# Francesco215/autoregressive_diffusion

Measured on AMD Instinct MI355X. Metric: denoiser-step frames/sec at 1/2/4/8 MI355X; 64-frame Lunar-Lander seq, higher is better.
Workload: dtype bf16; 1 GPU; Lunar-Lander 64-frame seq, gym EDM2 UNet 46.2M (gym_train.py:37-47), 8 seq/GPU (gym_train.py:55 micro_batch_size), step = EDM2Loss fwd + bwd + grad all-reduce + [grad-norm clip +] AdamW + 2 EMA profiles, 3:1 mix of 3-D/2-D steps; global_batch=8, seq_len=64, parallelism=dp1, hip_graph=False

## Files before the change

### autoregressive_diffusion_amd/_lib.py

```python
import ctypes as C
import os

import torch

_HERE = os.path.dirname(os.path.abspath(__file__))
LIB_PATH = os.path.join(_HERE, os.environ.get("ONIRIS_LIB_NAME", "liboniris_hip.so"))

if not os.path.exists(LIB_PATH):
    raise ImportError(f"{LIB_PATH} not found: build the HIP extension first (make -j8 at the repo root); "
                      "there is no CPU/PyTorch fallback for the denoiser kernels")

lib = C.CDLL(LIB_PATH)

c_void_p, c_int, c_float, c_int32, c_int64, c_size_t = C.c_void_p, C.c_int, C.c_float, C.c_int32, C.c_int64, C.c_size_t


class WeightDesc(C.Structure):
    _fields_ = [("w", c_void_p), ("grad", c_void_p), ("wf", c_void_p), ("wb", c_void_p), ("dwp", c_void_p), ("dws", c_void_p),
                ("cout", c_int32), ("cin", c_int32), ("taps", c_int32), ("kt", c_int32),
                ("CoutP", c_int32), ("CinP", c_int32), ("CoutPb", c_int32), ("CinPb", c_int32),
                ("row_start", c_int32), ("perm3", c_int32), ("gain", c_float), ("nsplit_cap", c_int32),
                ("nsplit", c_void_p), ("tile_start", c_int32), ("pad_", c_int32)]


class ConvArgs(C.Structure):
    _fields_ = [("x", c_void_p), ("ctx", c_void_p), ("w_own", c_void_p), ("w_ctx", c_void_p), ("out", c_void_p),
                ("coef_own", c_void_p), ("coef_ctx", c_void_p),
                ("B", c_int32), ("S", c_int32), ("T", c_int32), ("H", c_int32), ("W", c_int32),
                ("Cin", c_int32), ("CinP", c_int32), ("Cout", c_int32), ("CoutP", c_int32), ("taps", c_int32),
                ("ctx_bstride", c_int32), ("ctx_T", c_int32), ("coff0", c_int32), ("coff1", c_int32),
                ("ctx_fill", c_float), ("epi", c_int32),
                ("res", c_void_p), ("escale", c_void_p), ("emb_gain", c_void_p), ("out2", c_void_p),
                ("ta", c_float), ("tb", c_float), ("clip", c_float), ("ctx_out", c_void_p),
                ("big_tile", c_int32), ("escale_pitch", c_int32),
                ("splitk_ws", c_void_p), ("splitk_ws_bytes", C.c_size_t), ("clip_flag", c_void_p),
                ("ctx_prod", c_void_p), ("ctx_prod_mode", c_int32), ("x_split", c_int32), ("x2", c_void_p), ("act_out", c_void_p),
                ("cat_w1", c_float), ("cat_w2", c_float), ("ctx_rows", c_int32)]


class WgradArgs(C.Structure):
    _fields_ = [("x", c_void_p), ("dy", c_void_p), ("dwp", c_void_p), ("scale", c_void_p),
                ("B", c_int32), ("T", c_int32), ("H", c_int32), ("W", c_int32), ("Cin", c_int32), ("CinP", c_int32),
                ("Cout", c_int32), ("CoutP", c_int32), ("taps", c_int32),
                ("xb_stride", c_int32), ("x_T", c_int32), ("coff", c_int32), ("fill", c_float),
                ("nsplit_cap", c_int32), ("taps_total", c_int32), ("tap0", c_int32), ("pad_", c_int32),
                ("nsplit_out", c_void_p)]


class AttnArgs(C.Structure):
    _fields_ = [("q", c_void_p), ("k", c_void_p), ("v", c_void_p), ("qt", c_void_p), ("kt", c_void_p),
                ("vt", c_void_p), ("out", c_void_p), ("lse", c_void_p),
                ("kv_num", c_void_p), ("kv_idx", c_void_p), ("q_num", c_void_p), ("q_idx", c_void_p),
                ("tab_cols", c_int32), ("qtab_cols", c_int32),
                ("B", c_int32), ("heads", c_int32), ("Lq", c_int32), ("Lk", c_int32), ("C", c_int32),
                ("mask_mode", c_int32), ("P", c_int32), ("T", c_int32), ("tab_block", c_int32),
                ("dout", c_void_p), ("doutt", c_void_p), ("delta", c_void_p),
                ("dq", c_void_p), ("dk", c_void_p), ("dv", c_void_p),
                ("dkv_part", c_void_p), ("dkv_chunks", c_int32), ("dkv_item_keys", c_int32),
                ("sched", c_void_p), ("sched_wgs", c_int32), ("sched_slots", c_int32), ("v_bstride", c_int64),
                ("k_bstride", c_int64), ("split_ws", c_void_p), ("kv_splits", c_int32), ("frame_kernel", c_int32)]


class AttnF32Args(C.Structure):
    _fields_ = [("q", c_void_p), ("k", c_void_p), ("v", c_void_p), ("out", c_void_p), ("lse", c_void_p),
                ("dout", c_void_p), ("delta", c_void_p), ("dq", c_void_p), ("dk", c_void_p), ("dv", c_void_p),
                ("BH", c_int32), ("Lq", c_int32), ("Lk", c_int32), ("D", c_int32), ("mask_mode", c_int32), ("P", c_int32),
                ("T", c_int32), ("q_frame_off", c_int32), ("scale", c_float), ("pad_", c_int32)]


EPI_NONE, EPI_EMB_SILU, EPI_MPSUM = 0, 1, 2

_SIGS = {
    "oniris_last_error": (C.c_char_p, []),
    "oniris_abi_version": (c_int, []),
    "oniris_struct_sizes": (c_int, [c_void_p]),
    "oniris_profile_arm": (c_int, [c_void_p, c_void_p]),
    "oniris_profile_disarm": (c_int, []),
    "oniris_set_cu_reserve": (c_int, [c_int]),
    "oniris_set_ew_nt_bytes": (c_int64, [c_int64]),
    "oniris_frame_attn_bwd": (c_int, [c_void_p, c_void_p]),
    "oniris_frame_attn_qkv_fwd": (c_int, [c_void_p, c_void_p, c_void_p, c_int64, c_int, c_int, c_void_p]),
    "oniris_frame_attn_qkv_bwd": (c_int, [c_void_p, c_void_p, c_void_p, c_void_p, c_void_p, c_int64, c_int, c_int, c_void_p]),
    "oniris_conv_f32": (c_int, [c_void_p, c_void_p, c_void_p, c_int64, c_int, c_int, c_int, c_int, c_int, c_void_p]),
    "oniris_wgrad_f32": (c_int, [c_void_p, c_void_p, c_void_p, c_int64, c_int, c_int, c_int, c_int, c_int, c_void_p]),
    "oniris_attn_f32_fwd": (c_int, [c_void_p, c_void_p]),
    "oniris_attn_f32_bwd": (c_int, [c_void_p, c_void_p]),
    "oniris_census": (c_int, [c_int]),
    "oniris_census_read": (c_int64, [C.c_char_p, c_int64]),
    "oniris_train_mask": (c_int, [c_int, c_int, c_void_p, c_void_p, C.POINTER(c_int)]),
    "oniris_infer_mask": (c_int, [c_int, c_int, c_void_p, c_void_p, C.POINTER(c_int)]),
    "oniris_mask_transpose": (c_int, [c_int, c_int, c_void_p, c_void_p, c_void_p, c_void_p]),
    "oniris_attn_schedule": (c_int, [c_int, c_int, c_void_p, c_int, c_void_p, c_int]),
    "oniris_weight_prep": (c_int, [c_void_p, c_int, c_int, c_int, c_int, c_void_p]),
# ... 131 lines not shown
```

### autoregressive_diffusion_amd/csrc/common.h

```cpp
#pragma once
#include <hip/hip_runtime.h>
#include <hip/hip_ext.h>
#include <stdint.h>
#include <stdio.h>
#include <string.h>

typedef __bf16 bf16;
typedef __attribute__((ext_vector_type(8))) __bf16 bf16x8;
typedef __attribute__((ext_vector_type(4))) __bf16 bf16x4;
typedef __attribute__((ext_vector_type(2))) __bf16 bf16x2;
typedef __attribute__((ext_vector_type(4))) short s16x4;
typedef __attribute__((ext_vector_type(16))) float f32x16;
typedef __attribute__((ext_vector_type(4))) float f32x4;
typedef __attribute__((ext_vector_type(4))) unsigned int u32x4;

#define ONIRIS_OK 0
#define ONIRIS_EINVAL (-1)
#define ONIRIS_ELAUNCH (-2)
#define ONIRIS_EUNSUPPORTED (-3)

void oniris_set_error(const char* fmt, ...);

#define ONIRIS_CHECK_ARG(cond, ...)                \
  do {                                             \
// ... 46 lines not shown
}
template <bool NT, typename V>
__device__ __forceinline__ void stv(V* p, V v) {
  if constexpr (NT) __builtin_nontemporal_store(v, p);
  else *p = v;
}

extern int oniris_cu_reserve;
int oniris_persistent_wgs(void);

static inline int cdiv(int a, int b) { return (a + b - 1) / b; }
static inline int roundup(int a, int b) { return cdiv(a, b) * b; }

#ifdef __HIPCC__
__device__ __forceinline__ float bf2f(bf16 v) { return (float)v; }
__device__ __forceinline__ bf16 f2bf(float v) { return (bf16)v; }

__device__ __forceinline__ f32x16 mfma32(bf16x8 a, bf16x8 b, f32x16 c) {
  return __builtin_amdgcn_mfma_f32_32x32x16_bf16(a, b, c, 0, 0, 0);
}
__device__ __forceinline__ float sigmoid_fast(float z) {
  return __builtin_amdgcn_rcpf(1.f + __builtin_amdgcn_exp2f(-1.4426950408889634f * z));
}
__device__ __forceinline__ int mfma_row(int r, int lane) { return (r & 3) + 8 * (r >> 2) + 4 * (lane >> 5); }

__device__ __forceinline__ float wave_sum(float v) {
#pragma unroll
  for (int o = 32; o > 0; o >>= 1) v += __shfl_xor(v, o);
  return v;
}
__device__ __forceinline__ float wave_max(float v) {
#pragma unroll
  for (int o = 32; o > 0; o >>= 1) v = fmaxf(v, __shfl_xor(v, o));
  return v;
}

__device__ __forceinline__ float block_sum(float v, float* red) {
  v = wave_sum(v);
  const int w = threadIdx.x >> 6, nw = blockDim.x >> 6;
  __syncthreads();
  if ((threadIdx.x & 63) == 0) red[w] = v;
  __syncthreads();
  float t = 0.f;
  for (int i = 0; i < nw; ++i) t += red[i];
  return t;
}
// ... 2 lines not shown
```

### autoregressive_diffusion_amd/csrc/conv1x1_glds.h

```cpp
#pragma once
#include "conv_kernels.h"
#include "lds_dma.h"

struct C1Cfg {
  static constexpr int BM = 256, BN = 128, CK = 64, NW = 8, NTHR = 512, NSTG = 3;
  static constexpr int STG = (BM + BN) * 128;
  static constexpr int NPA = BM * 8 / NTHR, NPW = BN * 8 / NTHR;
  static constexpr int EROW = 64 * 2 + 16;
  static_assert(NW * 32 * EROW <= STG, "the epilogue stages through one (free) stage buffer");
  static_assert(NSTG * STG <= 160 * 1024, "stages must fit the LDS");
};

__global__ __launch_bounds__(512, 1) void conv1x1_glds_kernel(const ConvDev d) {
#if defined(__HIP_DEVICE_COMPILE__)
  using Cfg = C1Cfg;
  constexpr int BM = Cfg::BM, BN = Cfg::BN, CK = Cfg::CK, NTHR = Cfg::NTHR, STG = Cfg::STG, NSTG = Cfg::NSTG;
  constexpr int NPA = Cfg::NPA, NPW = Cfg::NPW, EROW = Cfg::EROW;
  __shared__ __attribute__((aligned(16))) unsigned char smem[NSTG * STG];
  const OnirisConvArgs& a = d.a;
  const int tid = threadIdx.x, lane = tid & 63, wave = __builtin_amdgcn_readfirstlane(tid >> 6), r = lane & 31, h = lane >> 5;
  const int wp = wave & 3, wc = wave >> 2;
  const int Cin = a.Cin, Cout = a.Cout;
  const long long M = (long long)a.B * a.S * a.T * a.H * a.W;
  const int nchunk = Cin / CK, ncb = d.ncob, ntiles = d.ntt * ncb;
// ... 101 lines not shown
      const long long prow = m0 + wp * 64 + m * 32;
      auto put = [&](int nt, const float (&v)[16]) __attribute__((always_inline)) {
#pragma unroll
        for (int g = 0; g < 4; ++g) {
          bf16x4 o;
#pragma unroll
          for (int k = 0; k < 4; ++k) o[k] = f2bf(v[4 * g + k]);
          *(bf16x4*)(ep + r * EROW + (nt * 32 + 8 * g + 4 * h) * 2) = o;
        }
      };
      auto flush = [&](bf16* dst) __attribute__((always_inline)) {
#pragma unroll
        for (int it = 0; it < 4; ++it) {
          const int id = it * 64 + lane, row = id >> 3, part = id & 7;
          const int co = cow + part * 8;
          if (prow + row < M && co < Cout) {
            const u32x4 v_ = *(const u32x4*)(ep + row * EROW + part * 16);
            u32x4* o_ = (u32x4*)(dst + (size_t)(prow + row) * Cout + co);
            if (d.nt) __builtin_nontemporal_store(v_, o_); else *o_ = v_;
          }
        }
      };
      float v[16];
      if (a.epi == ONIRIS_EPI_MPSUM) {
        if (a.out2) {
#pragma unroll
          for (int nt = 0; nt < 2; ++nt) {
#pragma unroll
            for (int i = 0; i < 16; ++i) v[i] = acc[m][nt][i];
            put(nt, v);
          }
          flush((bf16*)a.out2);
        }
        const bool valid = prow + r < M;
        const size_t obase = (size_t)(prow + r) * Cout;
#pragma unroll
        for (int nt = 0; nt < 2; ++nt) {
#pragma unroll
          for (int g = 0; g < 4; ++g) {
            const int co = cow + nt * 32 + 8 * g + 4 * h;
            bf16x4 rv;
#pragma unroll
            for (int k = 0; k < 4; ++k) rv[k] = f2bf(0.f);
            if (valid && co < Cout) rv = *(const bf16x4*)((const bf16*)a.res + obase + co);
#pragma unroll
            for (int k = 0; k < 4; ++k) {
              float o = a.ta * bf2f(rv[k]) + a.tb * acc[m][nt][4 * g + k];
// ... 2 lines not shown
            }
          }
          put(nt, v);
        }
        flush(og);
      } else {
#pragma unroll
        for (int nt = 0; nt < 2; ++nt) {
#pragma unroll
          for (int i = 0; i < 16; ++i) v[i] = acc[m][nt][i];
          put(nt, v);
        }
        flush(og);
      }
    }
    drained = true;
  }
#endif
}

static inline bool conv1x1_glds_ok(const OnirisConvArgs& a) {
  const long long M = (long long)a.B * a.S * a.T * a.H * a.W;
  return a.taps == 1 && !a.ctx && a.Cin % 64 == 0 && a.CinP == a.Cin && a.Cin <= 1024 && a.Cout % 8 == 0 &&
         (a.epi == ONIRIS_EPI_NONE || a.epi == ONIRIS_EPI_MPSUM) && M >= 8192 && M * a.Cin * 2 < (1LL << 31) &&
         (long long)a.CoutP * a.CinP * 2 < (1LL << 31);
}

static int launch_conv1x1_glds(const OnirisConvArgs& a, hipStream_t stream) {
  ConvDev d;
  d.a = a;
  const long long M = (long long)a.B * a.S * a.T * a.H * a.W;
  d.ntt = (int)((M + C1Cfg::BM - 1) / C1Cfg::BM);
  d.ncob = cdiv(a.CoutP, C1Cfg::BN);
  d.ntx = d.nty = 1; d.ksplit = 1; d.reduce = 0;
  d.nt = M * a.Cout * 2 >= oniris_ew_nt_bytes();
  const long long ntiles = (long long)d.ntt * d.ncob;
  const int ncu = oniris_persistent_wgs();
  const long long nblk = ntiles < ncu ? ntiles : ncu;
  oniris_launch_tagged(d.nt ? "nt-stores" : nullptr, conv1x1_glds_kernel, dim3((unsigned)nblk), dim3(C1Cfg::NTHR), stream, d);
  ONIRIS_LAUNCH_CHECK();
  return ONIRIS_OK;
}
```

### autoregressive_diffusion_amd/csrc/conv_api.hip

```cpp
#include "conv_fwd_common.h"

extern "C" int oniris_conv_fwd(const OnirisConvArgs* args, oniris_stream_t stream_) {
  hipStream_t st = (hipStream_t)stream_;
  ONIRIS_CHECK_ARG(args && args->w_own && ((args->x && args->out) || args->ctx_prod_mode == 3), "conv_fwd: null pointer");
  const OnirisConvArgs& a = *args;
  if (a.ctx_prod_mode != 0 && !(a.S == 1 && a.ctx && a.taps == 9 && a.ctx_prod)) {
    oniris_set_error("conv_fwd: ctx_prod_mode %d is for the one-frame cached evaluation (S == 1, context path, ctx_prod given)", a.ctx_prod_mode);
    return ONIRIS_EUNSUPPORTED;
  }
  if (a.ctx_rows != 0 && !(a.S == 1 && a.T == 1 && a.ctx && a.taps == 9 && a.ctx_rows > 0 && a.B == 2 * a.ctx_rows &&
                           a.ctx_out == nullptr && a.ctx_prod_mode != 3)) {
    oniris_set_error("conv_fwd: ctx_rows %d is for the one-frame cached evaluation of a guided pair (S = T = 1, context path, "
                     "B = 2 * ctx_rows (got B = %d), no ctx_out, ctx_prod_mode != 3)", a.ctx_rows, a.B);
    return ONIRIS_EUNSUPPORTED;
  }
  ONIRIS_CHECK_ARG(a.taps == 9 || a.taps == 1, "conv_fwd: taps must be 1 or 9 (got %d)", a.taps);
  ONIRIS_CHECK_ARG(a.B > 0 && a.T > 0 && a.H > 0 && a.W > 0 && (a.S == 1 || a.S == 2), "conv_fwd: bad sizes");
  ONIRIS_CHECK_ARG(a.Cin % 8 == 0 && a.Cout % 8 == 0, "conv_fwd: Cin, Cout must be multiples of 8 (%d,%d)", a.Cin, a.Cout);
  ONIRIS_CHECK_ARG(a.CoutP % 32 == 0 && a.CinP % 64 == 0 && a.CoutP >= a.Cout && a.CinP >= a.Cin,
                   "conv_fwd: bad padded sizes CoutP=%d CinP=%d", a.CoutP, a.CinP);
  ONIRIS_CHECK_ARG(a.epi != ONIRIS_EPI_MPSUM || a.res, "conv_fwd: EPI_MPSUM needs res");
  ONIRIS_CHECK_ARG(a.epi != ONIRIS_EPI_EMB_SILU || (a.escale && a.out2), "conv_fwd: EPI_EMB_SILU needs escale/out2");
  ONIRIS_CHECK_ARG(a.x2 == nullptr || (a.taps == 1 && a.ctx == nullptr), "conv_fwd: x2 (concatenated input) is a 1x1, context-free option");
  const bool has_ctx = a.ctx != nullptr;
  ONIRIS_CHECK_ARG(!has_ctx || (a.w_ctx && a.taps == 9), "conv_fwd: context path needs w_ctx and taps == 9");
  if (a.clip_flag && (a.taps == 1 || (a.S == 1 && has_ctx))) {
    const hipError_t e = hipMemsetD32Async((hipDeviceptr_t)a.clip_flag, 1, 1, st);
    if (e != hipSuccess) { oniris_set_error("conv: clip_flag fill failed: %s", hipGetErrorString(e)); return ONIRIS_ELAUNCH; }
  }
  if (a.taps == 1) {
    ONIRIS_CHECK_ARG(a.S == 1, "conv_fwd: 1x1 variant expects S == 1 (fold slots into T)");
    return conv_dispatch_1x1(a, st);
  }
  if (a.S == 2) {
    ONIRIS_CHECK_ARG(has_ctx, "conv_fwd: S == 2 is the DART training layout and needs the context path");
    return conv_dispatch_s2ctx(a, st);
  }
  return has_ctx ? conv_dispatch_s1ctx(a, st) : conv_dispatch_s1(a, st);
}
```

### autoregressive_diffusion_amd/csrc/conv_kernels.h

```cpp
#pragma once
#include <type_traits>
#include <cstdlib>
#include "common.h"
#include "../../include/oniris.h"

template <int PW_, int NPOS_ = 128>
struct Patch {
  static constexpr int PW = PW_;
  static constexpr int NPOS = NPOS_;
  static constexpr int PH = (PW_ == 16) ? (NPOS_ / 16) : PW_;
  static constexpr int FT = NPOS_ / (PW * PH);
  static constexpr int HW = PW + 2, HH = PH + 2;
  static constexpr int HALO = FT * HH * HW;
};

struct ConvDev {
  OnirisConvArgs a;
  int ntx, nty, ntt, ncob;
  int grid3d;
  int ksplit;
  int reduce;
  int nt;
};

template <int S, int TAPS, int CK, int NT, bool HAS_CTX, int PW, int NW = 4>
struct ConvCfg {
  using P = Patch<PW, 32 * NW>;
// ... 319 lines not shown
  unsigned char* ep = smem + wave * 32 * EROW;
  auto flush = [&](bf16* dst, size_t blk) __attribute__((always_inline)) {
    constexpr int PO = BN / 8;
#pragma unroll
    for (int it = 0; it < 32 * PO / 64; ++it) {
      const int id = it * 64 + lane;
      const int row = id / PO, part = id % PO;
      const int pr = wave * 32 + row;
      bool ok;
      size_t px_;
      if constexpr (TAPS == 9) {
        const int f_ = pr / (P::PH * P::PW), yy = (pr / P::PW) % P::PH, xx = pr % P::PW;
        ok = (t0 + f_) < T;
        px_ = (size_t)(t0 + f_) * HWp + (y0 + yy) * W + (x0 + xx);
      } else {
        ok = (q0 + pr) < T * HWp;
        px_ = (size_t)(q0 + pr);
      }
      const int co = co0 + part * 8;
      if (ok && co < a.Cout) *(uint4*)(dst + (blk + px_) * a.Cout + co) = *(const uint4*)(ep + row * EROW + part * 16);
    }
  };
  bf16* og = (bf16*)a.out;
#pragma unroll
  for (int s = 0; s < S; ++s) {
    const int n = (b * S + s) * T + tloc;
    const float cown = (a.coef_own && valid) ? a.coef_own[n] : 1.f;
    float cctx = 0.f;
    if constexpr (HAS_CTX) cctx = (a.coef_ctx && valid) ? a.coef_ctx[n] : 1.f;
    const size_t blk = (size_t)(b * S + s) * T * HWp;
    const size_t obase = (blk + pix) * a.Cout;
    float v[NT][16];
#pragma unroll
    for (int nt = 0; nt < NT; ++nt)
#pragma unroll
      for (int i = 0; i < 16; ++i) {
        v[nt][i] = cown * acc[s][nt][i];
        if constexpr (HAS_CTX) v[nt][i] = __builtin_fmaf(cctx, accc[nt][i], v[nt][i]);
      }
    auto stage = [&]() __attribute__((always_inline)) {
#pragma unroll
      for (int nt = 0; nt < NT; ++nt)
#pragma unroll
        for (int g = 0; g < 4; ++g) {
          bf16x4 o;
#pragma unroll
          for (int k = 0; k < 4; ++k) o[k] = f2bf(v[nt][4 * g + k]);
          *(bf16x4*)(ep + pr * EROW + (nt * 32 + 8 * g + 4 * h) * 2) = o;
        }
    };
    if (a.epi == ONIRIS_EPI_MPSUM) {
      if (a.out2) { stage(); flush((bf16*)a.out2, blk); }
#pragma unroll
      for (int nt = 0; nt < NT; ++nt)
#pragma unroll
        for (int g = 0; g < 4; ++g) {
          const int co = co0 + nt * 32 + 8 * g + 4 * h;
          bf16x4 rv;
#pragma unroll
          for (int k = 0; k < 4; ++k) rv[k] = f2bf(0.f);
          if (valid && co < a.Cout) rv = *(const bf16x4*)((const bf16*)a.res + obase + co);
#pragma unroll
          for (int k = 0; k < 4; ++k) {
            float o = a.ta * bf2f(rv[k]) + a.tb * v[nt][4 * g + k];
            if (a.clip > 0.f) o = fminf(fmaxf(o, -a.clip), a.clip);
            v[nt][4 * g + k] = o;
          }
        }
    }
    stage();
    flush(og, blk);
    if (a.epi == ONIRIS_EPI_EMB_SILU) {
#pragma unroll
// ... 73 lines not shown
```

### autoregressive_diffusion_amd/csrc/elementwise.hip

```cpp
#include <cstdlib>
#include "common.h"
#include "../../include/oniris.h"

#define SILU_SCALE (1.0f / 0.596f)

__device__ __forceinline__ float silu_f(float z) { return z * sigmoid_fast(z); }
__device__ __forceinline__ float dsilu_f(float z) {
  const float sg = sigmoid_fast(z);
  return sg * (1.f + z * (1.f - sg));
}

template <bool NORM, bool NT>
__global__ __launch_bounds__(256) void act_fwd_kernel(const bf16* __restrict__ x, const bf16* __restrict__ skip,
                                                      bf16* __restrict__ xo, bf16* __restrict__ a,
                                                      float* __restrict__ sden, long long npix, int C1, int C2, float w1,
                                                      float w2, int rs, int Ho, int Wo) {
  const int C = C1 + C2, G = C >> 3;
  const long long gid = (long long)blockIdx.x * 256 + threadIdx.x;
  const long long pix = gid / G;
  const int cg = (int)(gid % G);
  const bool ok = pix < npix;
  float v[8];
#pragma unroll
  for (int i = 0; i < 8; ++i) v[i] = 0.f;
  if (ok) {
    const int c = cg * 8;
    bf16x8 in;
    float w;
    if (c < C1) {
      w = w1;
      if (rs == 0) in = ldv<NT>((const bf16x8*)(x + pix * C1 + c));
      else {
        const int xo_ = (int)(pix % Wo), yo_ = (int)((pix / Wo) % Ho);
// ... 945 lines not shown
```

### autoregressive_diffusion_amd/edm2/networks_edm2.py

```python
import inspect
import math
from contextlib import nullcontext
import torch
from torch import nn
import torch.nn.functional as F

from .. import ops
from .. import fp32 as _fp32
from .loss_weight import MultiNoiseLoss
from .utils import BetterModule, MPFourier, to_cl, from_cl, BF16, strip_runtime_state
from .conv import MPConv, MPCausal3DGatedConv, Gating, weights_ready, batched_gates
from .attention import FrameAttention, VideoAttention


def unwrap_ddp(m):
    return m.module if isinstance(m, torch.nn.parallel.DistributedDataParallel) else m


class Block(nn.Module):
    def __init__(self, in_channels, out_channels, emb_channels, flavor="enc", resample_mode="keep",
                 resample_filter=[1, 1], attention=False, channels_per_head=64, dropout=0, res_balance=0.3,
                 attn_balance=0.3, clip_act=256):
        super().__init__()
        self._taps = ops.resample_taps(resample_filter)
# ... 11 lines not shown
        else:
            self.attn = FrameAttention(out_channels, self.num_heads, attn_balance)

    __getstate__ = strip_runtime_state

    def _cl(self, x, emb, batch_size, c_noise, cache=None, update_cache=False, just_2d=False, skip=None, cat_w=None,
            c=None, in_slot=None, skip_slot=None, private_out=False, pair=False):
        if cache is None:
            cache = {}
        rs = self.resample_mode
        if rs != "keep" and (self._taps is not None or skip is not None or (self.flavor == "enc" and self.conv_skip is not None)):
            x, in_slot, rs = ops.resample(x, rs, in_slot, self._taps), None, "keep"
        skip_conv_done = False
        want_xs = (private_out and ops.ALIAS2 and self.training and torch.is_grad_enabled()
                   and not (self.flavor == "dec" and self.conv_skip is not None))
        if self.flavor == "enc" and self.conv_skip is not None:
            x, in_slot = self.conv_skip._cl(x, in_slot=in_slot), None
        xs = ops.GradSlot() if (want_xs and (x.requires_grad or (skip is not None and skip.requires_grad))) else None
        if self.flavor == "enc":
            x, a = ops.act(x, norm=True, in_slot=in_slot, resample=rs, xo_slot=xs)
        elif (skip is not None and self.conv_skip is not None and not self.training
              and ops.conv_cat_act_ok(x, skip, self.conv_skip.weight.pw)):
            x, a = ops.conv_cat_act(x, skip, cat_w[0], cat_w[1], self.conv_skip.weight.pw)
            skip_conv_done = True
        elif skip is not None:
            x, a = ops.act(x, skip, cat_w[0], cat_w[1], want_xo=True, in_slot=in_slot, skip_slot=skip_slot, xo_slot=xs)
        else:
            x, a = ops.act(x, want_xo=True, in_slot=in_slot, resample=rs, xo_slot=xs)
        N = x.shape[0]
        if c is None:
            c = (self.emb_linear._cl(emb).reshape(N, -1).float() * self.emb_gain + 1)
        pk = dict(pair=True) if pair else {}
        y, cache["conv_res0"] = self.conv_res0._cl(a, batch_size, c_noise, cache.get("conv_res0"), update_cache,
                                                   just_2d, cscale=c, **pk)
        if self.training and self.dropout != 0:
            y = F.dropout(y, p=self.dropout)
        if self.flavor == "dec" and self.conv_skip is not None and not skip_conv_done:
            x = self.conv_skip._cl(x)
        t = self.res_balance
        den = 1.0 / math.sqrt((1 - t) ** 2 + t ** 2)
        clip = float(self.clip_act) if self.clip_act is not None else 0.0
        x, cache["conv_res1"] = self.conv_res1._cl(y, batch_size, c_noise, cache.get("conv_res1"), update_cache, just_2d,
                                                   res=x, ta=(1 - t) * den, tb=t * den,
                                                   clip=clip if self.num_heads == 0 else 0.0,
                                                   grad_private=private_out, **pk,
                                                   **(dict(res_slot=xs, res_alias=True) if xs is not None else {}))
# ... 411 lines not shown
```

### autoregressive_diffusion_amd/ops.py

```python
import ctypes
import math
import numpy as np
import torch

from . import _lib
from ._lib import lib, check

BF16 = torch.bfloat16


_raw_stream = getattr(torch._C, "_cuda_getCurrentRawStream", None)


def _stream():
    if _raw_stream is not None:
        return ctypes.c_void_p(_raw_stream(torch.cuda.current_device()))
    return ctypes.c_void_p(torch.cuda.current_stream().cuda_stream)


def _p(t):
    return None if t is None else t.data_ptr()


def _need_gpu(*ts):
# ... 480 lines not shown
    return 16 if W >= 16 else W


def _s2ctx_family(T, H, W, Cin, CinP, CoutP, ctx_T, coff, ctx_fill):
    ok = ctx_fill in (0.0, 1.0)
    if (BIG_TILE >= 4 and ok and Cin == 32 and CinP == 64 and CoutP == 32 and W % 16 == 0 and H % 4 == 0 and ctx_T == T
            and tuple(coff) in ((-2, -1), (2, 1))):
        return "stream"
    if BIG_TILE >= 3 and ok and Cin % 32 == 0 and H % 16 == 0 and W % 16 == 0:
        return "glds16"
    if BIG_TILE >= 3 and ok and Cin % 32 == 0 and H == 8 and W == 8 and CoutP % 64 == 0:
        return "glds8"
    return "staged"


PROFILE_SHAPES = int(_os.environ.get("ONIRIS_PROFILE_SHAPES", "0"))
ALIAS2 = int(_os.environ.get("ONIRIS_ALIAS2", "1"))
CLIP_FLAG = int(_os.environ.get("ONIRIS_CLIP_FLAG", "1"))


def _conv_launch(x, ctx, w_own, w_ctx, out, coef_own, coef_ctx, B, S, T, H, W, Cin, CinP, Cout, CoutP, taps,
                 ctx_bstride=0, ctx_T=0, coff=(0, 0), ctx_fill=0.0, epi=0, res=None, escale=None, emb_gain=None,
                 out2=None, ta=0.0, tb=0.0, clip=0.0, ctx_out=None, clip_flag=None, ctx_prod=None, ctx_prod_mode=0,
                 x2=None, act_out=None, x_split=0, cat_w=(1.0, 1.0), ctx_rows=0):
    if KernelProfile.enabled:
        flops = 2.0 * B * S * T * H * W * Cout * Cin * taps
        if ctx is not None:
            flops += 2.0 * B * T * H * W * Cout * Cin * 2 * taps
        nt = 2 if CoutP % 64 == 0 else 1
        if (BIG_TILE >= 4 and S == 2 and ctx is not None and taps == 9 and Cin == 32 and CinP == 64 and CoutP == 32 and W % 16 == 0
                and H % 4 == 0 and ctx_fill in (0.0, 1.0) and ctx_T == T and tuple(coff) in ((-2, -1), (2, 1))):
            key = f"conv_stream_kernel<ALIAS={int(ctx.data_ptr() == x.data_ptr() and ctx_bstride == 2 * T and coff[0] < 0)}>"
        elif (BIG_TILE >= 3 and S == 2 and ctx is not None and taps == 9 and Cin % 32 == 0 and H % 16 == 0 and W % 16 == 0
                and ctx_fill in (0.0, 1.0)):
            key = f"conv_glds_kernel<NT={nt},PW=16,NW=8,MT=1,WC=1,CTX=1>"
        elif (BIG_TILE >= 3 and S == 2 and ctx is not None and taps == 9 and Cin % 32 == 0 and H == 8 and W == 8
              and CoutP % 64 == 0 and ctx_fill in (0.0, 1.0)):
            key = "conv_glds_kernel<NT=1,PW=8,NW=8,MT=1,WC=2,CTX=1>"
        elif (BIG_TILE >= 4 and not (BIG_TILE & 128) and S == 1 and ctx is None and taps == 9 and Cin == 32 and CinP == 64 and CoutP == 32
              and W % 16 == 0 and H % 8 == 0 and x2 is None and B * T * (H // 8) * (W // 16) >= 512):
            key = "conv_plain_stream_kernel"
        elif (BIG_TILE >= 3 and S == 1 and ctx is None and taps == 9 and Cin % 32 == 0 and T % 2 == 0
              and ((H % 16 == 0 and W % 16 == 0) or (H == 8 and W == 8 and CoutP % 64 == 0))):
            key = (f"conv_glds_kernel<NT={nt},PW=16,NW=8,MT=1,WC=1,CTX=0>" if H % 16 == 0 else
                   "conv_glds_kernel<NT=1,PW=8,NW=8,MT=1,WC=2,CTX=0>")
        elif (BIG_TILE >= 3 and taps == 1 and ctx is None and Cin % 64 == 0 and CinP == Cin and epi in (0, _lib.EPI_MPSUM)
              and B * S * T * H * W >= 8192):
            key = "conv1x1_glds_kernel"
        else:
            key = f"conv_fwd_kernel<S={S},TAPS={taps},CK={32 if taps == 9 else 64},NT={nt},CTX={int(ctx is not None)},PW={_patch_w(W)}>"
        if PROFILE_SHAPES:
            key += f" [{H}x{W} {Cin}->{Cout} epi={epi}{' res' if res is not None else ''}{' out2' if out2 is not None else ''}{' y3' if ctx_out is not None else ''}{' dgrad' if coff[0] > 0 else ''}]"
        KernelProfile.enabled = False
        try:
            e0, e1 = _timed_launch(lambda: _conv_launch(x, ctx, w_own, w_ctx, out, coef_own, coef_ctx, B, S, T, H, W, Cin, CinP,
                                                        Cout, CoutP, taps, ctx_bstride, ctx_T, coff, ctx_fill, epi, res, escale,
                                                        emb_gain, out2, ta, tb, clip, ctx_out, clip_flag, ctx_prod, ctx_prod_mode,
                                                        ctx_rows=ctx_rows))
        finally:
            KernelProfile.enabled = True
        px = B * T * H * W
        nbytes = 2.0 * (S * px * Cin + S * px * Cout * (1 + (out2 is not None) + (res is not None))
                        + (px * Cout if ctx_out is not None else 0)
                        + taps * CoutP * CinP * (3 if ctx is not None else 1))
        if ctx is not None and ctx.data_ptr() != x.data_ptr():
            nbytes += 2.0 * B * ctx_T * H * W * Cin
        KernelProfile.records.append((key, flops, e0, e1, nbytes))
        return
    a = _lib.ConvArgs()
    a.x, a.ctx, a.w_own, a.w_ctx, a.out = _p(x), _p(ctx), _p(w_own), _p(w_ctx), _p(out)
    a.coef_own, a.coef_ctx = _p(coef_own), _p(coef_ctx)
    a.B, a.S, a.T, a.H, a.W = B, S, T, H, W
    a.Cin, a.CinP, a.Cout, a.CoutP, a.taps = Cin, CinP, Cout, CoutP, taps
    a.ctx_bstride, a.ctx_T, a.coff0, a.coff1, a.ctx_fill = ctx_bstride, ctx_T, coff[0], coff[1], ctx_fill
    a.epi, a.res, a.escale, a.emb_gain, a.out2 = epi, _p(res), _p(escale), _p(emb_gain), _p(out2)
    if escale is not None:
        a.escale_pitch = escale.stride(0)
    a.ta, a.tb, a.clip, a.ctx_out = ta, tb, clip, _p(ctx_out)
    a.clip_flag = _p(clip_flag)
    a.ctx_prod, a.ctx_prod_mode = _p(ctx_prod), ctx_prod_mode
    if x2 is not None:
        a.x2, a.act_out, a.x_split, a.cat_w1, a.cat_w2 = _p(x2), _p(act_out), x_split, cat_w[0], cat_w[1]
    a.big_tile = BIG_TILE
    a.ctx_rows = ctx_rows
    if SPLITK and B * S * T * H * W <= 64 * 256 and ctx_prod_mode == 0 and ctx_rows == 0:
        ws = _splitk_workspace(x.device)
        a.splitk_ws, a.splitk_ws_bytes = _p(ws), ws.numel() * 4
    check(lib.oniris_conv_fwd(ctypes.byref(a), _stream()), "conv_fwd")


SPLITK = int(_os.environ.get("ONIRIS_SPLITK", "1"))
_splitk_cache = {}


def _splitk_workspace(device):
    key = str(device)
    if key not in _splitk_cache:
        _splitk_cache[key] = torch.empty(8 << 20, dtype=torch.float32, device=device)
    return _splitk_cache[key]


def _wgrad_args(x, dy, pw, scale, B, T, H, W, Cin, CinP, Cout, CoutP, taps, xb_stride, x_T, coff, fill, tap0=0):
    a = _lib.WgradArgs()
    pw.touched = pw.hit = True
    if pw.members is not None:
# ... 500 lines not shown
        dxo = dxo.contiguous() if dxo is not None else None
        dx = torch.empty(xshape, dtype=BF16, device=xo.device)
        dskip = torch.empty(sshape, dtype=BF16, device=xo.device) if C2 else None
        dadd = in_slot.take() if in_slot is not None else None
        if dadd is not None:
            dadd = dadd.contiguous()
            assert tuple(dadd.shape) == (tuple(xin_shape) if rs else tuple(dx.shape))
        check(lib.oniris_act_bwd(_p(da), _p(dxo), _p(xo), _p(sden), _p(dx), _p(dskip), _p(None if rs else dadd), npix, C1, C2,
                                 w1, w2, int(norm), dxo_scale, _stream()), "act_bwd")
        if rs:
            N_, Ho, Wo = xshape[0], xshape[1], xshape[2]
            dpre = torch.empty(xin_shape, dtype=BF16, device=xo.device)
            if rs == 1:
                check(lib.oniris_resample(_p(dx), _p(dpre), _p(dadd), N_, Ho, Wo, C1, 1, 0.25, _stream()), "resample")
            else:
                check(lib.oniris_resample(_p(dx), _p(dpre), _p(dadd), N_, Ho, Wo, C1, 0, 4.0, _stream()), "resample")
            dx = dpre
        if skip_slot is not None and dskip is not None:
            skip_slot.put(dskip)
            dskip = None
        return dx, dskip, None, None, None, None, None, None, None, None


def act(x, skip=None, w1=1.0, w2=1.0, norm=False, want_xo=False, in_slot=None, skip_slot=None, resample="keep", xo_slot=None):
    rs = {"keep": 0, "down": 1, "up": 2}[resample]
    return _ActFn.apply(x, skip, float(w1), float(w2), bool(norm), bool(want_xo), in_slot, skip_slot, rs, xo_slot)


def resample_taps(f):
    f = [float(v) for v in f]
    if len(f) < 2 or len(f) > 8 or len(f) % 2 != 0:
        raise NotImplementedError(f"resample filter {f}: an even number of taps, 2 .. 8")
    tot = sum(f)
    if tot == 0:
        raise ValueError(f"resample filter {f} sums to zero")
    t = tuple(v / tot for v in f)
    return None if t == (0.5, 0.5) else t


def _resample_launch(src, dst, add, N, H, W, C, mode, scale, taps):
    if taps is None:
        check(lib.oniris_resample(_p(src), _p(dst), _p(add), N, H, W, C, mode, scale, _stream()), "resample")
    else:
        arr = (ctypes.c_float * len(taps))(*taps)
        check(lib.oniris_resample_filter(_p(src), _p(dst), _p(add), N, H, W, C, mode, arr, len(taps), scale, _stream()),
              "resample_filter")
# ... 1011 lines not shown
```

### include/oniris.h

```cpp
#ifndef ONIRIS_H
#define ONIRIS_H
#include <stddef.h>
#include <stdint.h>

#ifdef __cplusplus
extern "C" {
#endif

typedef void* oniris_stream_t;

const char* oniris_last_error(void);
int oniris_abi_version(void);
int oniris_profile_arm(void* start_event, void* stop_event);
int oniris_profile_disarm(void);
int oniris_set_cu_reserve(int k);
long long oniris_set_ew_nt_bytes(long long bytes);
int oniris_census(int on);
long long oniris_census_read(char* buf , long long cap);
int oniris_struct_sizes(int32_t* out4 );

int oniris_train_mask(int n_frames, int image_size, int32_t* kv_num_blocks, int32_t* kv_indices, int* block_size);
int oniris_infer_mask(int n_frames, int image_size, int32_t* kv_num_blocks, int32_t* kv_indices, int* block_size);
int oniris_mask_transpose(int n_rows, int n_cols, const int32_t* kv_num_blocks, const int32_t* kv_indices,
                          int32_t* q_num_blocks, int32_t* q_indices);
// ... 49 lines not shown
                 oniris_stream_t stream);

int oniris_gates_bwd(const float* c_noise, const float* params, const int32_t* nctx, const float* dca, const float* dcb,
                     float* dparams, int L, int N, int T, oniris_stream_t stream);
int oniris_emb_scale(const void* c_all, const float* gain, const int32_t* seg, float* c, int N, int Ctot,
                     oniris_stream_t stream);
#define ONIRIS_EMB_BWD_CHUNKS 16
int oniris_emb_scale_bwd(const float* dc, const void* c_all, const float* gain, const int32_t* start, void* dc_all,
                         float* dgain_part, int N, int Ctot, int K, oniris_stream_t stream);
int oniris_embed_pre(const float* c_noise, const int64_t* labels, const float* freqs, const float* phases, void* four,
                     void* onehot, int N, int cnoise, int cnoiseP, int label_dim, int labelP, oniris_stream_t stream);
int oniris_embed_post(const void* e1, const void* e2, void* emb, size_t n, float t, oniris_stream_t stream);
int oniris_embed_post_bwd(const void* demb, const void* e1, const void* e2, void* de1, void* de2, size_t n, float t,
                          oniris_stream_t stream);

int oniris_adamw(float* p, const float* g, float* m, float* v, size_t n, float lr, float beta1, float beta2,
                 float eps, float weight_decay, int step, float grad_scale, oniris_stream_t stream);
int oniris_adamw_clip_ema(float* p, const float* g, float* m, float* v, size_t n, float lr, float beta1, float beta2,
                          float eps, float weight_decay, int step, float grad_scale, const float* gnorm_sq,
                          float max_norm, float* ema0, float ema_w0, float* ema1, float ema_w1, oniris_stream_t stream);
#define ONIRIS_SQNORM_WS 1024
int oniris_sqnorm(const float* g, size_t n, float* out, oniris_stream_t stream);

enum { ONIRIS_EPI_NONE = 0, ONIRIS_EPI_EMB_SILU = 1, ONIRIS_EPI_MPSUM = 2 };

typedef struct OnirisConvArgs {
  const void* x;
  const void* ctx;
  const void* w_own;
  const void* w_ctx;
  void* out;
  const float* coef_own;
  const float* coef_ctx;
  int32_t B, S, T, H, W;
  int32_t Cin, CinP, Cout, CoutP;
  int32_t taps;
  int32_t ctx_bstride, ctx_T, coff0, coff1;
  float ctx_fill;
  int32_t epi;
  const void* res;
  const void* escale;
  const float* emb_gain;
  void* out2;
  float ta, tb, clip;
  void* ctx_out;
  int32_t big_tile;
  int32_t escale_pitch;
  float* splitk_ws;
  size_t splitk_ws_bytes;
  int32_t* clip_flag;
  float* ctx_prod;
  int32_t ctx_prod_mode;
  int32_t x_split;
  const void* x2;
  void* act_out;
  float cat_w1, cat_w2;
  int32_t ctx_rows;
} OnirisConvArgs;

int oniris_conv_fwd(const OnirisConvArgs* args , oniris_stream_t stream);

typedef struct OnirisWgradArgs {
  const void* x;
  const void* dy;
  void* dwp;
  const float* scale;
  int32_t B, T, H, W, Cin, CinP, Cout, CoutP, taps;
  int32_t xb_stride, x_T, coff;
  float fill;
  int32_t nsplit_cap, taps_total, tap0;
  int32_t pad_;
  int32_t* nsplit_out;
} OnirisWgradArgs;

int oniris_conv_wgrad(const OnirisWgradArgs* args , oniris_stream_t stream);
int oniris_conv_wgrad_group(const OnirisWgradArgs* args , int ngroups,
                            oniris_stream_t stream);

int oniris_gconv_bwd_prep(const void* dout, const void* out, const void* y3, const float* coef_own,
                          const float* coef_ctx, float* d_coef_own, float* d_coef_ctx, void* dy3, int B, int S, int T,
// ... 129 lines not shown
```

Before: 8749 latent-frames/s.

## Fuse decoder-head activation backward into the 1x1 skip-conv dgrad epilogue

```diff
diff --git a/autoregressive_diffusion_amd/_lib.py b/autoregressive_diffusion_amd/_lib.py
--- a/autoregressive_diffusion_amd/_lib.py
+++ b/autoregressive_diffusion_amd/_lib.py
@@ -35,7 +35,8 @@
                 ("big_tile", c_int32), ("escale_pitch", c_int32),
                 ("splitk_ws", c_void_p), ("splitk_ws_bytes", C.c_size_t), ("clip_flag", c_void_p),
                 ("ctx_prod", c_void_p), ("ctx_prod_mode", c_int32), ("x_split", c_int32), ("x2", c_void_p), ("act_out", c_void_p),
-                ("cat_w1", c_float), ("cat_w2", c_float), ("ctx_rows", c_int32)]
+                ("cat_w1", c_float), ("cat_w2", c_float), ("ctx_rows", c_int32),
+                ("act_da", c_void_p), ("act_xo", c_void_p), ("act_dadd", c_void_p)]
 
 
 class WgradArgs(C.Structure):
@@ -68,7 +69,7 @@
                 ("T", c_int32), ("q_frame_off", c_int32), ("scale", c_float), ("pad_", c_int32)]
 
 
-EPI_NONE, EPI_EMB_SILU, EPI_MPSUM = 0, 1, 2
+EPI_NONE, EPI_EMB_SILU, EPI_MPSUM, EPI_ACT_BWD = 0, 1, 2, 3
 
 _SIGS = {
     "oniris_last_error": (C.c_char_p, []),
diff --git a/autoregressive_diffusion_amd/csrc/common.h b/autoregressive_diffusion_amd/csrc/common.h
--- a/autoregressive_diffusion_amd/csrc/common.h
+++ b/autoregressive_diffusion_amd/csrc/common.h
@@ -92,6 +92,11 @@
 __device__ __forceinline__ float sigmoid_fast(float z) {
   return __builtin_amdgcn_rcpf(1.f + __builtin_amdgcn_exp2f(-1.4426950408889634f * z));
 }
+__device__ __forceinline__ float silu_f(float z) { return z * sigmoid_fast(z); }
+__device__ __forceinline__ float dsilu_f(float z) {
+  const float sg = sigmoid_fast(z);
+  return sg * (1.f + z * (1.f - sg));
+}
 __device__ __forceinline__ int mfma_row(int r, int lane) { return (r & 3) + 8 * (r >> 2) + 4 * (lane >> 5); }
 
 __device__ __forceinline__ float wave_sum(float v) {
diff --git a/autoregressive_diffusion_amd/csrc/conv1x1_glds.h b/autoregressive_diffusion_amd/csrc/conv1x1_glds.h
--- a/autoregressive_diffusion_amd/csrc/conv1x1_glds.h
+++ b/autoregressive_diffusion_amd/csrc/conv1x1_glds.h
@@ -147,7 +147,27 @@
         }
       };
       float v[16];
-      if (a.epi == ONIRIS_EPI_MPSUM) {
+      if (a.epi == ONIRIS_EPI_ACT_BWD) {
+        const int C1 = a.x_split, C2 = Cout - C1;
+#pragma unroll
+        for (int nt = 0; nt < 2; ++nt) {
+#pragma unroll
+          for (int i = 0; i < 16; ++i) v[i] = acc[m][nt][i];
+          put(nt, v);
+        }
+#pragma unroll
+        for (int it = 0; it < 4; ++it) {
+          const int id = it * 64 + lane, row = id >> 3, part = id & 7;
+          const int co = cow + part * 8;
+          if (prow + row < M && co < Cout) {
+            const u32x4 v_ = *(const u32x4*)(ep + row * EROW + part * 16);
+            const size_t p_ = (size_t)(prow + row);
+            u32x4* o_ = (u32x4*)((co < C1) ? og + p_ * C1 + co : (bf16*)a.out2 + p_ * C2 + (co - C1));
+            if (d.nt) __builtin_nontemporal_store(act_bwd_part<true>(a, v_, p_, co), o_);
+            else *o_ = act_bwd_part<false>(a, v_, p_, co);
+          }
+        }
+      } else if (a.epi == ONIRIS_EPI_MPSUM) {
         if (a.out2) {
 #pragma unroll
           for (int nt = 0; nt < 2; ++nt) {
@@ -196,7 +216,7 @@
 static inline bool conv1x1_glds_ok(const OnirisConvArgs& a) {
   const long long M = (long long)a.B * a.S * a.T * a.H * a.W;
   return a.taps == 1 && !a.ctx && a.Cin % 64 == 0 && a.CinP == a.Cin && a.Cin <= 1024 && a.Cout % 8 == 0 &&
-         (a.epi == ONIRIS_EPI_NONE || a.epi == ONIRIS_EPI_MPSUM) && M >= 8192 && M * a.Cin * 2 < (1LL << 31) &&
+         (a.epi == ONIRIS_EPI_NONE || a.epi == ONIRIS_EPI_MPSUM || a.epi == ONIRIS_EPI_ACT_BWD) && M >= 8192 && M * a.Cin * 2 < (1LL << 31) &&
          (long long)a.CoutP * a.CinP * 2 < (1LL << 31);
 }
 
diff --git a/autoregressive_diffusion_amd/csrc/conv_api.hip b/autoregressive_diffusion_amd/csrc/conv_api.hip
--- a/autoregressive_diffusion_amd/csrc/conv_api.hip
+++ b/autoregressive_diffusion_amd/csrc/conv_api.hip
@@ -22,6 +22,11 @@
   ONIRIS_CHECK_ARG(a.epi != ONIRIS_EPI_MPSUM || a.res, "conv_fwd: EPI_MPSUM needs res");
   ONIRIS_CHECK_ARG(a.epi != ONIRIS_EPI_EMB_SILU || (a.escale && a.out2), "conv_fwd: EPI_EMB_SILU needs escale/out2");
   ONIRIS_CHECK_ARG(a.x2 == nullptr || (a.taps == 1 && a.ctx == nullptr), "conv_fwd: x2 (concatenated input) is a 1x1, context-free option");
+  ONIRIS_CHECK_ARG(a.epi != ONIRIS_EPI_ACT_BWD ||
+                       (a.taps == 1 && a.S == 1 && !a.ctx && !a.x2 && !a.coef_own && a.act_da && a.act_xo && a.out2 &&
+                        a.x_split > 0 && a.x_split < a.Cout && a.x_split % 8 == 0),
+                   "conv_fwd: EPI_ACT_BWD is a 1x1, context-free, single-source launch with act_da / act_xo / out2 and a split "
+                   "inside (0, Cout), a multiple of 8");
   const bool has_ctx = a.ctx != nullptr;
   ONIRIS_CHECK_ARG(!has_ctx || (a.w_ctx && a.taps == 9), "conv_fwd: context path needs w_ctx and taps == 9");
   if (a.clip_flag && (a.taps == 1 || (a.S == 1 && has_ctx))) {
diff --git a/autoregressive_diffusion_amd/csrc/conv_kernels.h b/autoregressive_diffusion_amd/csrc/conv_kernels.h
--- a/autoregressive_diffusion_amd/csrc/conv_kernels.h
+++ b/autoregressive_diffusion_amd/csrc/conv_kernels.h
@@ -3,6 +3,39 @@
 #include <cstdlib>
 #include "common.h"
 #include "../../include/oniris.h"
+
+template <bool NT>
+__device__ __forceinline__ u32x4 act_bwd_part(const OnirisConvArgs& a, u32x4 dxo_raw, size_t p, int c) {
+#pragma clang fp contract(off)
+  const int C1 = a.x_split;
+  const bf16x8 d2 = __builtin_bit_cast(bf16x8, dxo_raw);
+  const bf16x8 xin = ldv<NT>((const bf16x8*)((const bf16*)a.act_xo + p * a.Cout + c));
+  const bf16x8 dain = ldv<NT>((const bf16x8*)((const bf16*)a.act_da + p * a.Cout + c));
+  float g[8];
+#pragma unroll
+  for (int i = 0; i < 8; ++i) {
+    const float z = bf2f(xin[i]);
+    const float sg = sigmoid_fast(z);
+    const float ds = sg * __builtin_fmaf(1.f - sg, z, 1.f);
+    g[i] = bf2f(dain[i]) * ds * (1.f / 0.596f);
+    g[i] = g[i] + bf2f(d2[i]);
+  }
+  bf16x8 o;
+  if (c < C1) {
+    if (a.act_dadd) {
+      const bf16x8 d3 = ldv<NT>((const bf16x8*)((const bf16*)a.act_dadd + p * C1 + c));
+#pragma unroll
+      for (int i = 0; i < 8; ++i) o[i] = f2bf(__builtin_fmaf(a.cat_w1, g[i], bf2f(d3[i])));
+    } else {
+#pragma unroll
+      for (int i = 0; i < 8; ++i) o[i] = f2bf(g[i] * a.cat_w1);
+    }
+  } else {
+#pragma unroll
+    for (int i = 0; i < 8; ++i) o[i] = f2bf(g[i] * a.cat_w2);
+  }
+  return __builtin_bit_cast(u32x4, o);
+}
 
 template <int PW_, int NPOS_ = 128>
 struct Patch {
@@ -368,6 +401,21 @@
     }
   };
   bf16* og = (bf16*)a.out;
+  auto flush_cat = [&](size_t blk) __attribute__((always_inline)) {
+    constexpr int PO = BN / 8;
+    const int C1 = a.x_split, C2 = a.Cout - a.x_split;
+#pragma unroll
+    for (int it = 0; it < 32 * PO / 64; ++it) {
+      const int id = it * 64 + lane;
+      const int row = id / PO, part = id % PO;
+      const size_t px_ = blk + (size_t)(q0 + wave * 32 + row);
+      const int co = co0 + part * 8;
+      if ((q0 + wave * 32 + row) < T * HWp && co < a.Cout) {
+        bf16* dst = (co < C1) ? og + px_ * C1 + co : (bf16*)a.out2 + px_ * C2 + (co - C1);
+        *(u32x4*)dst = act_bwd_part<false>(a, *(const u32x4*)(ep + row * EROW + part * 16), px_, co);
+      }
+    }
+  };
 #pragma unroll
   for (int s = 0; s < S; ++s) {
     const int n = (b * S + s) * T + tloc;
@@ -395,6 +443,13 @@
           *(bf16x4*)(ep + pr * EROW + (nt * 32 + 8 * g + 4 * h) * 2) = o;
         }
     };
+    if constexpr (TAPS == 1 && S == 1 && !HAS_CTX) {
+      if (a.epi == ONIRIS_EPI_ACT_BWD) {
+        stage();
+        flush_cat(blk);
+        continue;
+      }
+    }
     if (a.epi == ONIRIS_EPI_MPSUM) {
       if (a.out2) { stage(); flush((bf16*)a.out2, blk); }
 #pragma unroll
diff --git a/autoregressive_diffusion_amd/csrc/elementwise.hip b/autoregressive_diffusion_amd/csrc/elementwise.hip
--- a/autoregressive_diffusion_amd/csrc/elementwise.hip
+++ b/autoregressive_diffusion_amd/csrc/elementwise.hip
@@ -4,11 +4,6 @@
 
 #define SILU_SCALE (1.0f / 0.596f)
 
-__device__ __forceinline__ float silu_f(float z) { return z * sigmoid_fast(z); }
-__device__ __forceinline__ float dsilu_f(float z) {
-  const float sg = sigmoid_fast(z);
-  return sg * (1.f + z * (1.f - sg));
-}
 
 template <bool NORM, bool NT>
 __global__ __launch_bounds__(256) void act_fwd_kernel(const bf16* __restrict__ x, const bf16* __restrict__ skip,
diff --git a/autoregressive_diffusion_amd/edm2/networks_edm2.py b/autoregressive_diffusion_amd/edm2/networks_edm2.py
--- a/autoregressive_diffusion_amd/edm2/networks_edm2.py
+++ b/autoregressive_diffusion_amd/edm2/networks_edm2.py
@@ -57,6 +57,10 @@
         elif (skip is not None and self.conv_skip is not None and not self.training
               and ops.conv_cat_act_ok(x, skip, self.conv_skip.weight.pw)):
             x, a = ops.conv_cat_act(x, skip, cat_w[0], cat_w[1], self.conv_skip.weight.pw)
+            skip_conv_done = True
+        elif (skip is not None and self.conv_skip is not None and self.training and torch.is_grad_enabled()
+              and ops.dec_head_ok(x, skip, self.conv_skip.weight.pw)):
+            x, a = ops.dec_head(x, skip, cat_w[0], cat_w[1], self.conv_skip.weight.pw, in_slot=in_slot, skip_slot=skip_slot)
             skip_conv_done = True
         elif skip is not None:
             x, a = ops.act(x, skip, cat_w[0], cat_w[1], want_xo=True, in_slot=in_slot, skip_slot=skip_slot, xo_slot=xs)
diff --git a/autoregressive_diffusion_amd/ops.py b/autoregressive_diffusion_amd/ops.py
--- a/autoregressive_diffusion_amd/ops.py
+++ b/autoregressive_diffusion_amd/ops.py
@@ -526,7 +526,7 @@
 def _conv_launch(x, ctx, w_own, w_ctx, out, coef_own, coef_ctx, B, S, T, H, W, Cin, CinP, Cout, CoutP, taps,
                  ctx_bstride=0, ctx_T=0, coff=(0, 0), ctx_fill=0.0, epi=0, res=None, escale=None, emb_gain=None,
                  out2=None, ta=0.0, tb=0.0, clip=0.0, ctx_out=None, clip_flag=None, ctx_prod=None, ctx_prod_mode=0,
-                 x2=None, act_out=None, x_split=0, cat_w=(1.0, 1.0), ctx_rows=0):
+                 x2=None, act_out=None, x_split=0, cat_w=(1.0, 1.0), ctx_rows=0, act_da=None, act_xo=None, act_dadd=None):
     if KernelProfile.enabled:
         flops = 2.0 * B * S * T * H * W * Cout * Cin * taps
         if ctx is not None:
@@ -548,7 +548,7 @@
               and ((H % 16 == 0 and W % 16 == 0) or (H == 8 and W == 8 and CoutP % 64 == 0))):
             key = (f"conv_glds_kernel<NT={nt},PW=16,NW=8,MT=1,WC=1,CTX=0>" if H % 16 == 0 else
                    "conv_glds_kernel<NT=1,PW=8,NW=8,MT=1,WC=2,CTX=0>")
-        elif (BIG_TILE >= 3 and taps == 1 and ctx is None and Cin % 64 == 0 and CinP == Cin and epi in (0, _lib.EPI_MPSUM)
+        elif (BIG_TILE >= 3 and taps == 1 and ctx is None and Cin % 64 == 0 and CinP == Cin and epi in (0, _lib.EPI_MPSUM, _lib.EPI_ACT_BWD)
               and B * S * T * H * W >= 8192):
             key = "conv1x1_glds_kernel"
         else:
@@ -560,7 +560,8 @@
             e0, e1 = _timed_launch(lambda: _conv_launch(x, ctx, w_own, w_ctx, out, coef_own, coef_ctx, B, S, T, H, W, Cin, CinP,
                                                         Cout, CoutP, taps, ctx_bstride, ctx_T, coff, ctx_fill, epi, res, escale,
                                                         emb_gain, out2, ta, tb, clip, ctx_out, clip_flag, ctx_prod, ctx_prod_mode,
-                                                        ctx_rows=ctx_rows))
+                                                        x2=x2, act_out=act_out, x_split=x_split, cat_w=cat_w, ctx_rows=ctx_rows,
+                                                        act_da=act_da, act_xo=act_xo, act_dadd=act_dadd))
         finally:
             KernelProfile.enabled = True
         px = B * T * H * W
@@ -569,6 +570,8 @@
                         + taps * CoutP * CinP * (3 if ctx is not None else 1))
         if ctx is not None and ctx.data_ptr() != x.data_ptr():
             nbytes += 2.0 * B * ctx_T * H * W * Cin
+        if act_da is not None:
+            nbytes += 2.0 * px * (2 * Cout + (x_split if act_dadd is not None else 0))
         KernelProfile.records.append((key, flops, e0, e1, nbytes))
         return
     a = _lib.ConvArgs()
@@ -585,6 +588,8 @@
     a.ctx_prod, a.ctx_prod_mode = _p(ctx_prod), ctx_prod_mode
     if x2 is not None:
         a.x2, a.act_out, a.x_split, a.cat_w1, a.cat_w2 = _p(x2), _p(act_out), x_split, cat_w[0], cat_w[1]
+    if act_da is not None:
+        a.act_da, a.act_xo, a.act_dadd, a.x_split, a.cat_w1, a.cat_w2 = _p(act_da), _p(act_xo), _p(act_dadd), x_split, cat_w[0], cat_w[1]
     a.big_tile = BIG_TILE
     a.ctx_rows = ctx_rows
     if SPLITK and B * S * T * H * W <= 64 * 256 and ctx_prod_mode == 0 and ctx_rows == 0:
@@ -1131,6 +1136,62 @@
         return dx, dskip, None, None, None, None, None, None, None, None
 
 
+DEC_HEAD_FUSED = int(_os.environ.get("ONIRIS_DEC_HEAD_FUSED", "1"))
+
+
+class _DecHeadFn(torch.autograd.Function):
+
+    @staticmethod
+    def forward(ctx, x, skip, wparam, w1, w2, pw, in_slot, skip_slot):
+        _need_gpu(x)
+        x, skip = x.contiguous(), skip.contiguous()
+        N, H, W, C1 = x.shape
+        C2 = skip.shape[-1]
+        C = C1 + C2
+        npix = N * H * W
+        xo = torch.empty((N, H, W, C), dtype=BF16, device=x.device)
+        a = torch.empty_like(xo)
+        check(lib.oniris_act_fwd(_p(x), _p(skip), _p(xo), _p(a), None, npix, C1, C2, w1, w2, 0, 0, 0, 0, _stream()), "act_fwd")
+        Co = roundup(pw.cout, 8)
+        h = torch.empty((N, H, W, Co), dtype=BF16, device=x.device)
+        _conv_launch(xo, None, pw.wf, None, h, None, None, 1, 1, N, H, W, C, pw.CinP, Co, pw.CoutP, 1)
+        ctx.meta = (C1, C2, w1, w2, pw, in_slot, skip_slot)
+        ctx.save_for_backward(xo)
+        return h, a
+
+    @staticmethod
+    def backward(ctx, dh, da):
+        C1, C2, w1, w2, pw, in_slot, skip_slot = ctx.meta
+        xo, = ctx.saved_tensors
+        N, H, W, C = xo.shape
+        dh, da = dh.contiguous(), da.contiguous()
+        Co = dh.shape[-1]
+        dx = torch.empty((N, H, W, C1), dtype=BF16, device=xo.device)
+        dskip = torch.empty((N, H, W, C2), dtype=BF16, device=xo.device)
+        dadd = in_slot.take() if in_slot is not None else None
+        if dadd is not None:
+            dadd = dadd.contiguous()
+            assert tuple(dadd.shape) == tuple(dx.shape)
+        _conv_launch(dh, None, pw.wb, None, dx, None, None, 1, 1, N, H, W, Co, pw.CinPb, C, pw.CoutPb, 1,
+                     epi=_lib.EPI_ACT_BWD, out2=dskip, x_split=C1, cat_w=(w1, w2), act_da=da, act_xo=xo, act_dadd=dadd)
+        if _wants_wgrad(pw):
+            _wgrad_launch(xo, dh, pw, None, 1, N, H, W, C, pw.CinP, Co, pw.CoutP, 1, N, N, 0, 0.0)
+            pw.bank.request_finish()
+        if skip_slot is not None:
+            skip_slot.put(dskip)
+            dskip = None
+        return dx, dskip, None, None, None, None, None, None
+
+
+def dec_head_ok(x, skip, pw):
+    C1, C2 = x.shape[-1], skip.shape[-1]
+    return bool(DEC_HEAD_FUSED and x.is_cuda and pw.taps == 1 and pw.cin == C1 + C2 and C1 % 8 == 0 and C2 % 8 == 0)
+
+
+def dec_head(x, skip, w1, w2, pw, in_slot=None, skip_slot=None):
+    return _DecHeadFn.apply(x, skip, pw.param, float(w1), float(w2), pw, in_slot, skip_slot)
+
+
 def act(x, skip=None, w1=1.0, w2=1.0, norm=False, want_xo=False, in_slot=None, skip_slot=None, resample="keep", xo_slot=None):
     rs = {"keep": 0, "down": 1, "up": 2}[resample]
     return _ActFn.apply(x, skip, float(w1), float(w2), bool(norm), bool(want_xo), in_slot, skip_slot, rs, xo_slot)
diff --git a/include/oniris.h b/include/oniris.h
--- a/include/oniris.h
+++ b/include/oniris.h
@@ -95,7 +95,7 @@
 #define ONIRIS_SQNORM_WS 1024
 int oniris_sqnorm(const float* g, size_t n, float* out, oniris_stream_t stream);
 
-enum { ONIRIS_EPI_NONE = 0, ONIRIS_EPI_EMB_SILU = 1, ONIRIS_EPI_MPSUM = 2 };
+enum { ONIRIS_EPI_NONE = 0, ONIRIS_EPI_EMB_SILU = 1, ONIRIS_EPI_MPSUM = 2, ONIRIS_EPI_ACT_BWD = 3 };
 
 typedef struct OnirisConvArgs {
   const void* x;
@@ -129,6 +129,9 @@
   void* act_out;
   float cat_w1, cat_w2;
   int32_t ctx_rows;
+  const void* act_da;
+  const void* act_xo;
+  const void* act_dadd;
 } OnirisConvArgs;
 
 int oniris_conv_fwd(const OnirisConvArgs* args , oniris_stream_t stream);
```

Measured after the change: 8844 latent-frames/s (median of 6 runs). 1.01x the previous value.
